# JonasGeiping/breaching

Measured on NVIDIA H100. Metric: reconstruction iters/sec (ResNet-18 224x224, invertinggradients), higher is better.
Workload: dtype tf32

## Files before the change

breaching_b200/csrc/igemm_tc.cu:

```cuda
#include <stdlib.h>
#include <string.h>

#include <array>
#include <map>
#include <mutex>
#include <type_traits>

#include <cuda.h>

#include "igemm.cuh"

namespace bre {

namespace {

constexpr int TC_BM = 128;
constexpr int TC_BK = 32;
constexpr int TC_STAGES = 4;
constexpr int TC_MAX_STAGES = 8;
constexpr int TC_THREADS = 128;
constexpr int TC_BLOCK = 2 * TC_THREADS;

struct TcDims {
  int M, Nc, K;
// ... 88 lines not shown
template <int N>
__device__ __forceinline__ void cp_async_wait() { asm volatile("cp.async.wait_group %0;" ::"n"(N) : "memory"); }
__device__ __forceinline__ void cp_async_arrive(uint64_t* bar) {
  asm volatile("cp.async.mbarrier.arrive.noinc.shared::cta.b64 [%0];" ::"r"(smem_u32(bar)) : "memory");
}
__device__ __forceinline__ void consumer_sync() { asm volatile("bar.sync 1, %0;" ::"n"(TC_THREADS) : "memory"); }
__device__ __forceinline__ void cluster_sync_all() {
  asm volatile("barrier.cluster.arrive.release.aligned;" ::: "memory");
  asm volatile("barrier.cluster.wait.acquire.aligned;" ::: "memory");
}
__device__ __forceinline__ float4 ld_dsmem4(uint32_t saddr, uint32_t rank) {
  uint32_t raddr;
  asm("mapa.shared::cluster.u32 %0, %1, %2;" : "=r"(raddr) : "r"(saddr), "r"(rank));
  float4 v;
  asm volatile("ld.shared::cluster.v4.f32 {%0, %1, %2, %3}, [%4];" : "=f"(v.x), "=f"(v.y), "=f"(v.z), "=f"(v.w) : "r"(raddr));
  return v;
}

struct TcMaps {
  CUtensorMap act[2];
  CUtensorMap wgt[2];
};

constexpr int TC_MAXCLS = 4;
struct ClsPlan {
  int ncls, stride;
  int tile0[TC_MAXCLS + 1];
  int Hc[TC_MAXCLS], Wc[TC_MAXCLS], y0[TC_MAXCLS], x0[TC_MAXCLS];
  int Ty[TC_MAXCLS], Tx[TC_MAXCLS], Ly[TC_MAXCLS], Lx[TC_MAXCLS], ey[TC_MAXCLS], ex[TC_MAXCLS];
};
struct TcMapsCls {
  CUtensorMap act[2 * TC_MAXCLS];
  CUtensorMap wgt[2];
};

__device__ __forceinline__ void mbar_expect_tx(uint64_t* bar, uint32_t bytes) {
  asm volatile("mbarrier.arrive.expect_tx.shared::cta.b64 _, [%0], %1;" ::"r"(smem_u32(bar)), "r"(bytes) : "memory");
}
__device__ __forceinline__ void tma_im2col(uint32_t dst, const CUtensorMap* tm, uint64_t* bar, int c, int w, int h, int n, int ow, int oh) {
  asm volatile(
      "cp.async.bulk.tensor.4d.shared::cluster.global.im2col.mbarrier::complete_tx::bytes [%0], [%1, {%3, %4, %5, %6}], [%2], {%7, %8};"
      ::"r"(dst), "l"(reinterpret_cast<uint64_t>(tm)), "r"(smem_u32(bar)), "r"(c), "r"(w), "r"(h), "r"(n), "h"((uint16_t)ow), "h"((uint16_t)oh)
      : "memory");
}
__device__ __forceinline__ void tma_tile2d(uint32_t dst, const CUtensorMap* tm, uint64_t* bar, int c0, int c1) {
  asm volatile("cp.async.bulk.tensor.2d.shared::cluster.global.tile.mbarrier::complete_tx::bytes [%0], [%1, {%3, %4}], [%2];"
               ::"r"(dst), "l"(reinterpret_cast<uint64_t>(tm)), "r"(smem_u32(bar)), "r"(c0), "r"(c1) : "memory");
}
__device__ __forceinline__ void tma_tile3d(uint32_t dst, const CUtensorMap* tm, uint64_t* bar, int c0, int c1, int c2) {
  asm volatile("cp.async.bulk.tensor.3d.shared::cluster.global.tile.mbarrier::complete_tx::bytes [%0], [%1, {%3, %4, %5}], [%2];"
               ::"r"(dst), "l"(reinterpret_cast<uint64_t>(tm)), "r"(smem_u32(bar)), "r"(c0), "r"(c1), "r"(c2) : "memory");
}

template <int NV>
__device__ __forceinline__ void fused_bnact(const GemmEpilogue& e, long long row, int n, float (&v)[NV]) {
  const long long o = row + n;
#pragma unroll
  for (int j = 0; j < NV; ++j) {
    float u = v[j];
    if (e.kind == 1) {
      if (e.has_bn) u = fmaf(u, __ldg(e.scale + n + j), __ldg(e.shift + n + j));
      if (e.res != nullptr) u += e.res[o + j];
      u = e.relu ? fmaxf(u, 0.f) : u;
      v[j] = e.round_out ? tf32_rna(u) : u;
    } else {
      if (e.has_bn) {
        const float xhat = fmaf(e.pre[o + j], __ldg(e.inv + n + j), __ldg(e.nrm + n + j));
        u = fmaf(__ldg(e.scale + n + j), u, fmaf(__ldg(e.v_gamma + n + j), xhat, __ldg(e.v_beta + n + j)));
      }
      if (e.res != nullptr) u += e.res[o + j];
      if (e.relu && !(e.post[o + j] > 0.f)) u = 0.f;
      v[j] = e.round_out ? tf32_rna(u) : u;
    }
  }
}

#ifdef BRE_TC_TRACE
__device__ long long g_tc_trace[16];
#define TC_MARK(i, cond) do { if ((cond) && blockIdx.x == 0 && blockIdx.y == 0 && blockIdx.z == 0) g_tc_trace[i] = clock64(); } while (0)
#else
#define TC_MARK(i, cond) do { } while (0)
#endif

template <int MODE, int BN, bool TMA, bool CLS = false>
__global__ void __launch_bounds__(TC_BLOCK) igemm_tc_kernel(GemmArgs a, TcDims d, int proxy_fence,
                                                            const __grid_constant__ std::conditional_t<CLS, TcMapsCls, TcMaps> maps, ClsPlan plan) {
  static_assert(!CLS || (MODE == GEMM_DGRAD && TMA), "per-class gathers: strided dgrad with the TMA producer only");
  constexpr uint32_t A_BYTES = TC_BM * TC_BK * 4, B_BYTES = BN * TC_BK * 4;
  extern __shared__ __align__(1024) uint8_t smem[];
  uint8_t* sA = smem;
  const int nst = 1 << d.stage_shift, stage_mask = nst - 1;
  uint8_t* sB = smem + nst * A_BYTES;
  __shared__ __align__(8) uint64_t bar_full[TC_MAX_STAGES];
  __shared__ __align__(8) uint64_t bar_empty[TC_MAX_STAGES];

  TC_MARK(0, threadIdx.x == 0);
  pdl_launch_dependents();
  const ConvGeom g = a.g;
  const int tid = threadIdx.x, warp = tid >> 5, lane = tid & 31;
  const int ptid = tid & (TC_THREADS - 1);
  const bool consumer = warp < TC_THREADS / 32;
  const int n0 = blockIdx.y * BN, z = blockIdx.z;
  int m0 = blockIdx.x * TC_BM;
  int kb_begin = z * d.kblocks_per_split;
  int kb_end = min(d.total_kblocks, kb_begin + d.kblocks_per_split);
  const int HoWo = g.Ho * g.Wo, HW = g.H * g.W;
  int cls = 0, cHc = 0, cWc = 0, cTy = 0, cTx = 0, cls_kps = 0, Mrows = d.M;
  if (CLS) {
#pragma unroll
    for (int c = 1; c < TC_MAXCLS; ++c)
      if (c < plan.ncls && (int)blockIdx.x >= plan.tile0[c]) cls = c;
    m0 = ((int)blockIdx.x - plan.tile0[cls]) * TC_BM;
    cHc = plan.Hc[cls]; cWc = plan.Wc[cls]; cTy = plan.Ty[cls]; cTx = plan.Tx[cls];
    Mrows = g.N * cHc * cWc;
    cls_kps = cTy * cTx * (g.Co / TC_BK);
    const int total = cls_kps * a.nsrc, per = (total + (int)gridDim.z - 1) / (int)gridDim.z;
    kb_begin = z * per;
    kb_end = min(total, kb_begin + per);
  }

  if (tid == 0) {
#pragma unroll
    for (int s = 0; s < TC_MAX_STAGES; ++s) { mbar_init(&bar_full[s], TMA ? 1 : TC_THREADS); mbar_init(&bar_empty[s], TC_THREADS / 32); }
    fence_barrier_init();
  }
  __syncthreads();
  TC_MARK(1, threadIdx.x == 0);

  constexpr bool a_mn = MODE == GEMM_WGRAD;
  constexpr bool b_mn = MODE != GEMM_FPROP;

  constexpr int A_VEC = TC_BM * TC_BK / 4 / TC_THREADS;
  constexpr int B_VEC = BN * TC_BK / 4 / TC_THREADS;
  const int gcol = ptid & 7, grow = (ptid >> 3) & 15;
  int a_off[A_VEC];
  unsigned long long a_taps[A_VEC];
  int a_yx[A_VEC];
  if (!TMA && !consumer && (MODE == GEMM_FPROP || MODE == GEMM_DGRAD)) {
#pragma unroll
    for (int j = 0; j < A_VEC; ++j) {
      const int m = m0 + grow + 16 * j;
      a_off[j] = 0; a_taps[j] = 0ull; a_yx[j] = 0;
      if (m < d.M) {
        if (MODE == GEMM_FPROP) {
          const int img = m / HoWo, rem = m - img * HoWo;
          const int p = rem / g.Wo, q = rem - p * g.Wo;
          const int y0 = p * g.stride - g.pad, x0 = q * g.stride - g.pad;
          a_off[j] = (int)(img * a.x_sN) + (y0 * g.W + x0) * a.x_sP + gcol * 4;
          for (int r = 0; r < g.R; ++r)
            for (int s2 = 0; s2 < g.S; ++s2)
              if (y0 + r >= 0 && y0 + r < g.H && x0 + s2 >= 0 && x0 + s2 < g.W) a_taps[j] |= 1ull << (r * g.S + s2);
        } else {
          const int img = m / HW, rem = m - img * HW;
          const int y = rem / g.W, x = rem - y * g.W;
          const int yb = y + g.pad, xb = x + g.pad;
          const int py = yb / g.stride, qx = xb / g.stride;
          const int ey = yb - py * g.stride, ex = xb - qx * g.stride;
          a_off[j] = ((img * g.Ho + py) * g.Wo + qx) * g.Co + gcol * 4;
          a_yx[j] = (ey << 16) | ex;
          for (int r = ey, pp = py; r < g.R; r += g.stride, --pp)
            for (int s2 = ex, qq = qx; s2 < g.S; s2 += g.stride, --qq)
              if (pp >= 0 && pp < g.Ho && qq >= 0 && qq < g.Wo) a_taps[j] |= 1ull << (r * g.S + s2);
        }
      }
    }
  }
  int it_src, it_rs, it_c0;
  {
    const int kch = (MODE == GEMM_DGRAD) ? g.Co : g.Ci;
    it_src = kb_begin / d.kblocks_per_src;
    const int kbase = (kb_begin - it_src * d.kblocks_per_src) * TC_BK;
    it_rs = (MODE == GEMM_WGRAD) ? 0 : kbase / kch;
    it_c0 = (MODE == GEMM_WGRAD) ? kbase : kbase - it_rs * kch;
  }

  const int nkb = kb_end > kb_begin ? kb_end - kb_begin : 0;
  int base_n = 0, base_h = 0, base_w = 0;
  if (CLS) {
    const int per = cHc * cWc;
    base_n = m0 / per;
    const int rem = m0 - base_n * per;
    const int iy0 = rem / cWc, ix0 = rem - iy0 * cWc;
    base_h = iy0 + plan.Ly[cls]; base_w = ix0 + plan.Lx[cls];
  } else if (TMA && MODE != GEMM_WGRAD) {
    const int per = (MODE == GEMM_FPROP) ? HoWo : HW, wid = (MODE == GEMM_FPROP) ? g.Wo : g.W;
    base_n = m0 / per;
// ... 129 lines not shown
    const uint32_t pa = smem_u32(sA + stage * A_BYTES), pb = smem_u32(sB + stage * B_BYTES);
    if (MODE == GEMM_FPROP) {
      const int r = it_rs / g.S, s = it_rs - r * g.S;
      const int tapoff = (r * g.W + s) * a.x_sP + it_c0;
#pragma unroll
      for (int j = 0; j < A_VEC; ++j) {
        const bool ok = (a_taps[j] >> it_rs) & 1ull;
        cp_async16(pa + off_k128(grow + 16 * j, gcol), ok ? act + (a_off[j] + tapoff) : act, ok ? 16u : 0u);
      }
      const float* q = wgt + (long long)(n0 + grow) * d.K + kbase + gcol * 4;
#pragma unroll
      for (int j = 0; j < B_VEC; ++j) cp_async16(pb + off_k128(grow + 16 * j, gcol), q + (long long)(16 * j) * d.K, 16u);
    } else if (MODE == GEMM_DGRAD) {
      const int rs = it_rs, k0 = it_c0;
      const int r = rs / g.S, s = rs - r * g.S;
      if (g.stride == 1) {
        const int tapoff = k0 - (r * g.Wo + s) * g.Co;
#pragma unroll
        for (int j = 0; j < A_VEC; ++j) {
          const bool ok = (a_taps[j] >> rs) & 1ull;
          cp_async16(pa + off_k128(grow + 16 * j, gcol), ok ? act + (a_off[j] + tapoff) : act, ok ? 16u : 0u);
        }
      } else {
        const bool st2 = g.stride == 2;
#pragma unroll
        for (int j = 0; j < A_VEC; ++j) {
          const bool ok = (a_taps[j] >> rs) & 1ull;
          const int dr = r - (a_yx[j] >> 16), ds = s - (a_yx[j] & 0xffff);
          const int tr = st2 ? dr >> 1 : dr / g.stride, ts = st2 ? ds >> 1 : ds / g.stride;
          cp_async16(pa + off_k128(grow + 16 * j, gcol), ok ? act + (a_off[j] + k0 - (tr * g.Wo + ts) * g.Co) : act, ok ? 16u : 0u);
        }
      }
      const int n4 = ptid & 15, kk = ptid >> 4;
#pragma unroll
      for (int j = 0; j < B_VEC; ++j) {
        const int k = kk + 8 * j;
        const float* gb = wgt + ((long long)(k0 + k) * (g.R * g.S) + rs) * g.Ci + n0 + n4 * 4;
        cp_async16(pb + off_mn128(4 * n4, k), gb, 16u);
      }
    } else {
      {
        const int m4 = ptid & 31, kk = ptid >> 5;
#pragma unroll
        for (int j = 0; j < A_VEC; ++j) {
          const int k = kk + 4 * j;
          const int pix = kbase + k;
          const bool kok = pix < d.K;
          const bool mok = kok && (m0 + m4 * 4 < d.M);
          const float* ga = mok ? wgt + (long long)pix * g.Co + m0 + m4 * 4 : wgt;
          cp_async16(pa + off_mn128(4 * m4, k), ga, mok ? 16u : 0u);
        }
      }
      {
        const int n4 = ptid & 15, kk = ptid >> 4;
        const int n = n0 + n4 * 4;
        const int rs = n / g.Ci, c = n - rs * g.Ci;
        const int r = rs / g.S, s = rs - r * g.S;
#pragma unroll
        for (int j = 0; j < B_VEC; ++j) {
          const int k = kk + 8 * j;
          const int pix = kbase + k;
          bool ok = pix < d.K;
          const float* gb = act;
          if (ok) {
            const int img = pix / HoWo, rem = pix - img * HoWo;
            const int p = rem / g.Wo, q = rem - p * g.Wo;
            const int h = p * g.stride - g.pad + r, w = q * g.stride - g.pad + s;
            ok = h >= 0 && h < g.H && w >= 0 && w < g.W;
            if (ok) gb = act + img * a.x_sN + (long long)(h * g.W + w) * a.x_sP + c;
          }
          cp_async16(pb + off_mn128(4 * n4, k), gb, ok ? 16u : 0u);
        }
      }
    }
    it_c0 += TC_BK;
    if (MODE == GEMM_WGRAD) {
      if (it_c0 >= d.kblocks_per_src * TC_BK) { it_c0 = 0; ++it_src; }
    } else if (it_c0 >= kch) {
      it_c0 = 0;
      if (++it_rs == g.R * g.S) { it_rs = 0; ++it_src; }
    }
  };

  float acc[2][BN / 2];
#pragma unroll
  for (int h = 0; h < 2; ++h)
#pragma unroll
    for (int i = 0; i < BN / 2; ++i) acc[h][i] = 0.f;
  const int gq = lane >> 2, tq = lane & 3;
  if (consumer) {
    for (int i = 0; i < nkb; ++i) {
      const int stage = i & stage_mask;
      mbar_wait(&bar_full[stage], (uint32_t)((i >> d.stage_shift) & 1));
      TC_MARK(4, i == 0 && tid == 0);
      if constexpr (MODE == GEMM_FPROP) {
        if (!TMA || (proxy_fence & 1)) fence_proxy_async();
        const uint32_t sa = smem_u32(sA) + stage * A_BYTES, sb = smem_u32(sB) + stage * B_BYTES;
        wgmma_fence();
#pragma unroll
        for (int j = 0; j < TC_BK / 8; ++j) {
          const uint64_t db = wgmma_desc_k128(sb + 32 * j);
          wgmma_tf32<BN>(acc[0], wgmma_desc_k128(sa + 32 * j), db);
          wgmma_tf32<BN>(acc[1], wgmma_desc_k128(sa + 64 * 128 + 32 * j), db);
        }
        wgmma_commit();
        wgmma_wait<1>();
        fence_regs(acc[0]);
        fence_regs(acc[1]);
        __syncwarp();
        if (i > 0 && lane == 0) mbar_arrive(&bar_empty[(i - 1) & stage_mask]);
      } else {
        const uint8_t* pa = sA + stage * A_BYTES;
        const uint8_t* pb = sB + stage * B_BYTES;
#pragma unroll
        for (int j = 0; j < TC_BK / 8; ++j) {
          const int k0 = 8 * j + tq;
          uint32_t af[2][4];
#pragma unroll
          for (int h = 0; h < 2; ++h) {
            const int r = 64 * h + 16 * warp + gq;
            af[h][0] = ld_op<a_mn>(pa, r, k0);
            af[h][1] = ld_op<a_mn>(pa, r + 8, k0);
            af[h][2] = ld_op<a_mn>(pa, r, k0 + 4);
            af[h][3] = ld_op<a_mn>(pa, r + 8, k0 + 4);
          }
#pragma unroll
          for (int jn = 0; jn < BN / 8; ++jn) {
            const uint32_t b0 = ld_op<b_mn>(pb, 8 * jn + gq, k0), b1 = ld_op<b_mn>(pb, 8 * jn + gq, k0 + 4);
            mma_tf32(&acc[0][4 * jn], af[0], b0, b1);
            mma_tf32(&acc[1][4 * jn], af[1], b0, b1);
          }
        }
        __syncwarp();
        if (lane == 0) mbar_arrive(&bar_empty[stage]);
      }
    }
    if constexpr (MODE == GEMM_FPROP) {
      wgmma_wait<0>();
      fence_regs(acc[0]);
      fence_regs(acc[1]);
    }
    TC_MARK(5, tid == 0);
  } else {
    if (TMA) {
      if (producer) {
        KbState st = pst;
        for (int i = pw; i < nkb; i += nprod) {
          const int stage = i & stage_mask;
          if (i >= nst) mbar_wait(&bar_empty[stage], (uint32_t)(((i >> d.stage_shift) - 1) & 1));
          if (i >= nst || !((pre_wgt >> i) & 1u)) {
            mbar_expect_tx(&bar_full[stage], A_BYTES + B_BYTES);
            issue_wgt_tma(stage, st);
          }
          issue_act_tma(stage, st);
          TC_MARK(3, i == (nkb < nst ? nkb : nst) - 1);
          for (int u = 0; u < nprod; ++u) kb_advance(st);
        }
      }
      __syncwarp();
    } else {
      for (int i = 0; i < nkb; ++i) {
        const int stage = i & stage_mask;
        if (i >= nst) mbar_wait(&bar_empty[stage], (uint32_t)(((i >> d.stage_shift) - 1) & 1));
        issue_block(stage);
        cp_async_arrive(&bar_full[stage]);
      }
      cp_async_wait<0>();
    }
  }

  const int splits = gridDim.z;
  auto out_row = [&](int mm, long long& row, int& cs) {
    if (CLS) {
      const int per = cHc * cWc;
      const int img = mm / per, rem = mm - img * per;
      const int iy = rem / cWc, ix = rem - iy * cWc;
      row = img * a.x_sN + (long long)((plan.y0[cls] + plan.stride * iy) * g.W + plan.x0[cls] + plan.stride * ix) * a.x_sP;
      cs = a.x_sC;
    } else if (MODE == GEMM_DGRAD) {
      const int img = mm / HW;
      row = img * a.x_sN + (long long)(mm - img * HW) * a.x_sP;
      cs = a.x_sC;
    } else {
      row = (long long)mm * d.Nc;
      cs = 1;
    }
  };
  if (consumer && splits == 1) {
#pragma unroll
    for (int h = 0; h < 2; ++h) {
#pragma unroll
      for (int hr = 0; hr < 2; ++hr) {
        const int mm = m0 + 64 * h + 16 * warp + gq + 8 * hr;
        if (mm >= Mrows) continue;
        long long row;
        int cs;
        out_row(mm, row, cs);
#pragma unroll
        for (int jn = 0; jn < BN / 8; ++jn) {
          const int n = n0 + 8 * jn + 2 * tq;
          float v[2] = {acc[h][4 * jn + 2 * hr], acc[h][4 * jn + 2 * hr + 1]};
          if (MODE == GEMM_FPROP && a.bias != nullptr) {
            v[0] += __ldg(a.bias + n);
            v[1] += __ldg(a.bias + n + 1);
          }
          float* op = a.out + row + (long long)n * cs;
          if (MODE == GEMM_FPROP && a.epi.kind != 0) {
            if (a.out != nullptr) *reinterpret_cast<float2*>(op) = make_float2(v[0], v[1]);
            fused_bnact<2>(a.epi, row, n, v);
            *reinterpret_cast<float2*>(a.epi.out2 + row + n) = make_float2(v[0], v[1]);
          } else if (cs == 1) {
            float2 t2 = make_float2(v[0], v[1]);
            if (a.accumulate) {
              const float2 o = *reinterpret_cast<const float2*>(op);
              t2.x += o.x; t2.y += o.y;
            }
            *reinterpret_cast<float2*>(op) = t2;
          } else {
#pragma unroll
            for (int j = 0; j < 2; ++j) {
              float* q = op + (long long)j * cs;
              *q = a.accumulate ? *q + v[j] : v[j];
            }
          }
        }
      }
    }
  } else if (consumer) {
    consumer_sync();
    float* part = reinterpret_cast<float*>(sA);
#pragma unroll
    for (int h = 0; h < 2; ++h) {
#pragma unroll
      for (int hr = 0; hr < 2; ++hr) {
        const int r = 64 * h + 16 * warp + gq + 8 * hr;
#pragma unroll
        for (int jn = 0; jn < BN / 8; ++jn) {
          const int c = 8 * jn + 2 * tq;
          const int chunk = (c >> 2) ^ (r & (BN / 4 - 1) & 15);
          *reinterpret_cast<float2*>(part + r * BN + chunk * 4 + (c & 3)) = make_float2(acc[h][4 * jn + 2 * hr], acc[h][4 * jn + 2 * hr + 1]);
        }
      }
    }
  }
  if (splits > 1) {
    TC_MARK(7, tid == 0);
    cluster_sync_all();
    TC_MARK(8, tid == 0);
    if (consumer) {
      auto reduce_rows = [&](auto s_tag) {
        constexpr int S = decltype(s_tag)::value;
        constexpr int C4 = BN / 4, SLOTS = (TC_BM / S) * C4 / TC_THREADS > 0 ? (TC_BM / S) * C4 / TC_THREADS : 1;
        const uint32_t part_s = smem_u32(sA);
        float4 t[SLOTS][S];
        int rr[SLOTS], cc[SLOTS];
#pragma unroll
        for (int sl = 0; sl < SLOTS; ++sl) {
          const int slot = tid + sl * TC_THREADS;
          rr[sl] = z * (TC_BM / S) + slot / C4;
          cc[sl] = slot % C4;
          const uint32_t local = part_s + (uint32_t)(rr[sl] * BN + ((cc[sl] ^ (rr[sl] & (BN / 4 - 1) & 15)) << 2)) * 4u;
#pragma unroll
          for (int q = 0; q < S; ++q) t[sl][q] = ld_dsmem4(local, (uint32_t)q);
        }
#pragma unroll
        for (int sl = 0; sl < SLOTS; ++sl) {
          const int r = rr[sl], c4 = cc[sl];
          if (m0 + r >= Mrows) continue;
          float4 acc4 = t[sl][0];
#pragma unroll
          for (int q = 1; q < S; ++q) { acc4.x += t[sl][q].x; acc4.y += t[sl][q].y; acc4.z += t[sl][q].z; acc4.w += t[sl][q].w; }
          const int n = n0 + c4 * 4;
          if (MODE == GEMM_FPROP && a.bias != nullptr) {
            acc4.x += __ldg(a.bias + n); acc4.y += __ldg(a.bias + n + 1); acc4.z += __ldg(a.bias + n + 2); acc4.w += __ldg(a.bias + n + 3);
          }
          long long row;
          int cs;
          out_row(m0 + r, row, cs);
          float* op = a.out + row + (long long)n * cs;
          if (MODE == GEMM_FPROP && a.epi.kind != 0) {
            if (a.out != nullptr) *reinterpret_cast<float4*>(op) = acc4;
            float vv[4] = {acc4.x, acc4.y, acc4.z, acc4.w};
            fused_bnact<4>(a.epi, row, n, vv);
            *reinterpret_cast<float4*>(a.epi.out2 + row + n) = make_float4(vv[0], vv[1], vv[2], vv[3]);
          } else if (cs == 1) {
            if (a.accumulate) {
              const float4 o = *reinterpret_cast<const float4*>(op);
              acc4.x += o.x; acc4.y += o.y; acc4.z += o.z; acc4.w += o.w;
            }
            *reinterpret_cast<float4*>(op) = acc4;
          } else {
            const float vv[4] = {acc4.x, acc4.y, acc4.z, acc4.w};
#pragma unroll
            for (int j = 0; j < 4; ++j) {
              float* qq = op + (long long)j * cs;
              *qq = a.accumulate ? *qq + vv[j] : vv[j];
            }
          }
        }
      };
      switch (splits) {
        case 2: reduce_rows(std::integral_constant<int, 2>{}); break;
        case 4: reduce_rows(std::integral_constant<int, 4>{}); break;
        default: reduce_rows(std::integral_constant<int, 8>{}); break;
      }
    }
    TC_MARK(9, tid == 0);
    cluster_sync_all();
  }
  TC_MARK(10, tid == 0);
}

inline bool aligned16(const void* p) { return (reinterpret_cast<uintptr_t>(p) & 15) == 0; }

typedef CUresult (*EncodeIm2colFn)(CUtensorMap*, CUtensorMapDataType, cuuint32_t, void*, const cuuint64_t*, const cuuint64_t*, const int*,
                                   const int*, cuuint32_t, cuuint32_t, const cuuint32_t*, CUtensorMapInterleave, CUtensorMapSwizzle,
                                   CUtensorMapL2promotion, CUtensorMapFloatOOBfill);
typedef CUresult (*EncodeTiledFn)(CUtensorMap*, CUtensorMapDataType, cuuint32_t, void*, const cuuint64_t*, const cuuint64_t*,
                                  const cuuint32_t*, const cuuint32_t*, CUtensorMapInterleave, CUtensorMapSwizzle,
                                  CUtensorMapL2promotion, CUtensorMapFloatOOBfill);

struct TmaApi {
  EncodeIm2colFn im2col = nullptr;
  EncodeTiledFn tiled = nullptr;
  int driver = 0;
  bool ok = false;
};
const TmaApi& tma_api() {
  static const TmaApi api = [] {
    TmaApi t;
    cudaDriverEntryPointQueryResult q;
    void* f = nullptr;
    if (cudaGetDriverEntryPoint("cuTensorMapEncodeIm2col", &f, cudaEnableDefault, &q) == cudaSuccess && q == cudaDriverEntryPointSuccess)
      t.im2col = reinterpret_cast<EncodeIm2colFn>(f);
    f = nullptr;
    if (cudaGetDriverEntryPoint("cuTensorMapEncodeTiled", &f, cudaEnableDefault, &q) == cudaSuccess && q == cudaDriverEntryPointSuccess)
      t.tiled = reinterpret_cast<EncodeTiledFn>(f);
    cudaDriverGetVersion(&t.driver);
    t.ok = t.im2col != nullptr && t.tiled != nullptr;
    return t;
  }();
  return api;
}

using MapKey = std::array<long long, 16>;
std::mutex g_map_mutex;
std::map<MapKey, CUtensorMap> g_map_cache;

bool im2col_map(CUtensorMap* out, const float* base, int N, int H, int W, int C, long long sN, int sP, int lower_w, int lower_h,
                int upper_w, int upper_h, int stride, int chans, int pixels, CUtensorMapSwizzle swz) {
  const MapKey key = {0, (long long)reinterpret_cast<uintptr_t>(base), N, H, W, C, sN, sP, lower_w, lower_h, upper_w, upper_h, stride, chans,
                      pixels, (long long)swz};
  std::lock_guard<std::mutex> lock(g_map_mutex);
  auto it = g_map_cache.find(key);
  if (it != g_map_cache.end()) { *out = it->second; return true; }
  const TmaApi& api = tma_api();
  if (!api.ok) return false;
  const cuuint64_t dims[4] = {(cuuint64_t)C, (cuuint64_t)W, (cuuint64_t)H, (cuuint64_t)N};
  const cuuint64_t strides[3] = {(cuuint64_t)sP * 4, (cuuint64_t)W * sP * 4, (cuuint64_t)sN * 4};
  const int lower[2] = {lower_w, lower_h}, upper[2] = {upper_w, upper_h};
  const cuuint32_t estr[4] = {1, (cuuint32_t)stride, (cuuint32_t)stride, 1};
  CUtensorMap tm;
  const CUresult res = api.im2col(&tm, CU_TENSOR_MAP_DATA_TYPE_FLOAT32, 4, const_cast<float*>(base), dims, strides, lower, upper,
                                  (cuuint32_t)chans, (cuuint32_t)pixels, estr, CU_TENSOR_MAP_INTERLEAVE_NONE, swz,
                                  CU_TENSOR_MAP_L2_PROMOTION_L2_128B, CU_TENSOR_MAP_FLOAT_OOB_FILL_NONE);
  if (res != CUDA_SUCCESS) return false;
  g_map_cache.emplace(key, tm);
  *out = tm;
  return true;
}

bool tiled_map(CUtensorMap* out, const float* base, int rank, const long long* dims_ll, const long long* strides_elems, const int* box_i,
               CUtensorMapSwizzle swz) {
  MapKey key = {1, (long long)reinterpret_cast<uintptr_t>(base), rank, (long long)swz};
  for (int i = 0; i < rank; ++i) { key[4 + i] = dims_ll[i]; key[8 + i] = box_i[i]; if (i + 1 < rank) key[12 + i] = strides_elems[i]; }
  std::lock_guard<std::mutex> lock(g_map_mutex);
  auto it = g_map_cache.find(key);
  if (it != g_map_cache.end()) { *out = it->second; return true; }
  const TmaApi& api = tma_api();
  if (!api.ok) return false;
  cuuint64_t dims[3], strides[2];
  cuuint32_t box[3], estr[3] = {1, 1, 1};
  for (int i = 0; i < rank; ++i) { dims[i] = (cuuint64_t)dims_ll[i]; box[i] = (cuuint32_t)box_i[i]; }
  for (int i = 0; i + 1 < rank; ++i) strides[i] = (cuuint64_t)strides_elems[i] * 4;
  CUtensorMap tm;
  const CUresult res = api.tiled(&tm, CU_TENSOR_MAP_DATA_TYPE_FLOAT32, (cuuint32_t)rank, const_cast<float*>(base), dims, strides, box, estr,
                                 CU_TENSOR_MAP_INTERLEAVE_NONE, swz, CU_TENSOR_MAP_L2_PROMOTION_L2_128B, CU_TENSOR_MAP_FLOAT_OOB_FILL_NONE);
  if (res != CUDA_SUCCESS) return false;
  g_map_cache.emplace(key, tm);
  *out = tm;
  return true;
}

bool tma_eligible(const GemmArgs& a) {
  static const int tma_env = [] { const char* e = getenv("BRE_TC_TMA"); return e ? atoi(e) : 1; }();
  if (!tma_env || !tma_api().ok) return false;
  const ConvGeom& g = a.g;
  if (g.stride > 8 || g.pad > 127 || g.R - 1 - g.pad > 127 || g.S - 1 - g.pad > 127 || g.R > 128 || g.S > 128) return false;
  if (a.mode == GEMM_DGRAD) return g.stride == 1;
  if (a.mode == GEMM_WGRAD) return g.Ci % 32 == 0;
  return true;
}

bool build_maps(const GemmArgs& a, int BN, TcMaps* maps) {
  const ConvGeom& g = a.g;
  const CUtensorMapSwizzle K128 = CU_TENSOR_MAP_SWIZZLE_128B;
  for (int s = 0; s < a.nsrc; ++s) {
    if (a.mode == GEMM_FPROP) {
      if (!im2col_map(&maps->act[s], a.act[s], g.N, g.H, g.W, g.Ci, a.x_sN, a.x_sP, -g.pad, -g.pad, g.pad - (g.S - 1), g.pad - (g.R - 1),
                      g.stride, TC_BK, TC_BM, K128))
        return false;
      const long long K = (long long)g.R * g.S * g.Ci;
      const long long dims[2] = {K, g.Co}, strides[1] = {K};
      const int box[2] = {TC_BK, BN};
      if (!tiled_map(&maps->wgt[s], a.wgt[s], 2, dims, strides, box, K128)) return false;
    } else if (a.mode == GEMM_DGRAD) {
      const int lw = g.pad - (g.S - 1), lh = g.pad - (g.R - 1);
      if (!im2col_map(&maps->act[s], a.act[s], g.N, g.Ho, g.Wo, g.Co, (long long)g.Ho * g.Wo * g.Co, g.Co, lw, lh, lw + g.W - g.Wo,
                      lh + g.H - g.Ho, 1, TC_BK, TC_BM, K128))
        return false;
      const long long dims[3] = {g.Ci, (long long)g.R * g.S, g.Co}, strides[2] = {g.Ci, (long long)g.R * g.S * g.Ci};
      const int box[3] = {32, 1, TC_BK};
      if (!tiled_map(&maps->wgt[s], a.wgt[s], 3, dims, strides, box, K128)) return false;
    } else {
      const long long npix = (long long)g.N * g.Ho * g.Wo;
      const long long dims[2] = {g.Co, npix}, strides[1] = {g.Co};
      const int box[2] = {32, TC_BK};
      if (!tiled_map(&maps->wgt[s], a.wgt[s], 2, dims, strides, box, K128)) return false;
      if (!im2col_map(&maps->act[s], a.act[s], g.N, g.H, g.W, g.Ci, a.x_sN, a.x_sP, -g.pad, -g.pad, g.pad - (g.S - 1), g.pad - (g.R - 1),
                      g.stride, 32, TC_BK, K128))
        return false;
    }
  }
  return true;
}

struct AxisPlan { bool any; int y0, Hc, T, L, U; };
inline AxisPlan axis_plan(int H, int Ho, int R, int stride, int pad, int e) {
  AxisPlan p{false, 0, 0, 0, 0, 0};
  p.y0 = ((e - pad) % stride + stride) % stride;
  if (p.y0 >= H) return p;
  p.any = true;
  p.Hc = (H - p.y0 + stride - 1) / stride;
  if (e >= R) return p;
  p.T = (R - e + stride - 1) / stride;
  const int c = (p.y0 + pad - e) / stride;
  p.L = c - (p.T - 1);
  p.U = p.Hc - Ho + p.L;
  return p;
}

bool cls_eligible(const GemmArgs& a) {
  static const int env = [] { const char* e = getenv("BRE_TC_STRIDED_TMA"); return e ? atoi(e) : 1; }();
  const ConvGeom& g = a.g;
  if (!env || a.mode != GEMM_DGRAD || g.stride != 2 || !tma_api().ok) return false;
  static const int tma_env = [] { const char* e = getenv("BRE_TC_TMA"); return e ? atoi(e) : 1; }();
  if (!tma_env || g.R > 16 || g.S > 16) return false;
  for (int ey = 0; ey < 2; ++ey)
    for (int horiz = 0; horiz < 2; ++horiz) {
      const AxisPlan p = horiz ? axis_plan(g.W, g.Wo, g.S, 2, g.pad, ey) : axis_plan(g.H, g.Ho, g.R, 2, g.pad, ey);
      if (p.any && p.T > 0 && (p.L < -128 || p.L > 127 || p.U < -128 || p.U > 127)) return false;
    }
  return true;
}

bool build_cls(const GemmArgs& a, ClsPlan* plan, TcMapsCls* maps) {
  const ConvGeom& g = a.g;
  memset(plan, 0, sizeof(*plan));
  plan->stride = g.stride;
  int tiles = 0, n = 0;
  for (int ey = 0; ey < g.stride; ++ey) {
    const AxisPlan py = axis_plan(g.H, g.Ho, g.R, g.stride, g.pad, ey);
    if (!py.any) continue;
    for (int ex = 0; ex < g.stride; ++ex) {
      const AxisPlan px = axis_plan(g.W, g.Wo, g.S, g.stride, g.pad, ex);
      if (!px.any) continue;
      if (n >= TC_MAXCLS) return false;
      const bool taps = py.T > 0 && px.T > 0;
      plan->Hc[n] = py.Hc; plan->Wc[n] = px.Hc; plan->y0[n] = py.y0; plan->x0[n] = px.y0;
      plan->Ty[n] = taps ? py.T : 0; plan->Tx[n] = taps ? px.T : 0;
      plan->Ly[n] = py.L; plan->Lx[n] = px.L; plan->ey[n] = ey; plan->ex[n] = ex;
      plan->tile0[n] = tiles;
      tiles += ceil_div((long long)g.N * py.Hc * px.Hc, TC_BM);
      for (int s = 0; s < a.nsrc && taps; ++s)
        if (!im2col_map(&maps->act[2 * n + s], a.act[s], g.N, g.Ho, g.Wo, g.Co, (long long)g.Ho * g.Wo * g.Co, g.Co, px.L, py.L, px.U, py.U, 1,
                        TC_BK, TC_BM, CU_TENSOR_MAP_SWIZZLE_128B))
          return false;
      if (!taps)
        for (int s = 0; s < a.nsrc; ++s) maps->act[2 * n + s] = maps->act[s];
      ++n;
    }
  }
  plan->ncls = n;
  plan->tile0[n] = tiles;
  for (int s = 0; s < a.nsrc; ++s) {
    const long long dims[3] = {g.Ci, (long long)g.R * g.S, g.Co}, strides[2] = {g.Ci, (long long)g.R * g.S * g.Ci};
    const int box[3] = {32, 1, TC_BK};
    if (!tiled_map(&maps->wgt[s], a.wgt[s], 3, dims, strides, box, CU_TENSOR_MAP_SWIZZLE_128B)) return false;
  }
  return n > 0;
}

template <int MODE, int BN, bool TMA, bool CLS = false>
int launch_tc(const GemmArgs& a, const TcDims& d0, const std::conditional_t<CLS, TcMapsCls, TcMaps>& maps, cudaStream_t stream,
              const ClsPlan* plan_in = nullptr) {
  TcDims d = d0;
  ClsPlan plan;
  memset(&plan, 0, sizeof(plan));
  if (CLS) plan = *plan_in;
  const int tm = CLS ? plan.tile0[plan.ncls] : ceil_div(d.M, TC_BM), tn = d.Nc / BN;
  if (CLS) {
    int kmax = 0;
    for (int c = 0; c < plan.ncls; ++c) kmax = kmax > plan.Ty[c] * plan.Tx[c] ? kmax : plan.Ty[c] * plan.Tx[c];
    d.total_kblocks = kmax * (a.g.Co / TC_BK) * a.nsrc;
    if (d.total_kblocks < 1) d.total_kblocks = 1;
  }
  const long long tiles = (long long)tm * tn;
  static const int max_splits_env = [] { const char* e = getenv("BRE_TC_MAX_SPLITS"); return e ? atoi(e) : 0; }();
  static const int target_ctas_env = [] { const char* e = getenv("BRE_TC_TARGET_CTAS"); return e ? atoi(e) : 0; }();
  const int target = target_ctas_env > 0 ? target_ctas_env : kNumSMs;
  constexpr int kMaxCluster = 8;
  int splits = a.splits;
  if (splits <= 0) {
    splits = 1;
    while (splits < kMaxCluster && tiles * splits < target && d.total_kblocks / (splits * 2) >= 2) splits *= 2;
  }
  if (max_splits_env > 0 && splits > max_splits_env) splits = max_splits_env;
  int pow2 = 1;
  while (pow2 * 2 <= splits && pow2 < kMaxCluster) pow2 *= 2;
  splits = pow2;
  while (splits > 1 && splits > d.total_kblocks) splits /= 2;
  d.kblocks_per_split = ceil_div(d.total_kblocks, splits);
  if (tn > 65535) { set_error("igemm_tc: grid too large"); return -1; }
  static const int stages_env = [] { const char* e = getenv("BRE_TC_STAGES"); return e ? atoi(e) : 0; }();
  static const int shortk_env = [] { const char* e = getenv("BRE_TC_SHORTK_STAGES"); return e ? atoi(e) : 2; }();
  const bool shortk = shortk_env == 2 && d.kblocks_per_split <= 6 && tm == 1 && tiles * splits > 2LL * kNumSMs;
  const int stages = (stages_env == 8 || stages_env == 2) ? stages_env : (shortk ? 2 : TC_STAGES);
  d.stage_shift = stages == 8 ? 3 : (stages == 2 ? 1 : 2);
  const size_t smem = (size_t)stages * (TC_BM + BN) * TC_BK * 4;
  const size_t smem_max = (size_t)TC_MAX_STAGES * (TC_BM + BN) * TC_BK * 4;
  static bool attr_done = false;
  if (!attr_done) {
    BRE_CUDA_CHECK(cudaFuncSetAttribute(igemm_tc_kernel<MODE, BN, TMA, CLS>, cudaFuncAttributeMaxDynamicSharedMemorySize, (int)smem_max));
    attr_done = true;
  }
  static const int proxy_fence_env = [] {
    const char* e = getenv("BRE_TC_PROXY_FENCE");
    const char* pf = getenv("BRE_TC_PREFETCH");
    const char* np = getenv("BRE_TC_PRODUCERS");
    int nprod = np ? atoi(np) : 2;
    if (nprod < 1 || nprod > 4) nprod = 2;
    return (e && atoi(e) ? 1 : 0) | ((pf ? atoi(pf) : 1) ? 2 : 0) | (nprod << 2);
  }();
  {
    cudaError_t lerr = launch_kernel(igemm_tc_kernel<MODE, BN, TMA, CLS>, dim3(tm, tn, splits), dim3(TC_BLOCK), smem, stream, splits, a, d,
                                     proxy_fence_env, maps, plan);
    if (lerr != cudaSuccess) { set_error(std::string("igemm_tc launch failed: ") + cudaGetErrorString(lerr)); return -2; }
  }
  BRE_CHECK_LAUNCH();
  return 0;
}

}

static bool narrow_tiles_ok(const GemmArgs& a) {
  static const int env = [] { const char* e = getenv("BRE_TC_NARROW"); return e ? atoi(e) : 1; }();
  if (!env || !tma_eligible(a)) return false;
  if (a.mode == GEMM_DGRAD && a.g.stride != 1) return false;
  if (a.mode == GEMM_WGRAD && (a.g.Ci % 32 != 0)) return false;
  return true;
}

bool igemm_tc_supported(const GemmArgs& a) {
  const ConvGeom& g = a.g;
  int M, Nc, K;
  gemm_dims(a, M, Nc, K);
  for (int s = 0; s < a.nsrc; ++s)
    if (!aligned16(a.act[s]) || !aligned16(a.wgt[s])) return false;
  if (!aligned16(a.out) || (a.splits == 0 && a.ws == nullptr)) return false;
  const bool x_nhwc = a.x_sC == 1 && a.x_sP % 4 == 0 && a.x_sN % 4 == 0;
  if (Nc % 64 != 0 && !(Nc % 32 == 0 && narrow_tiles_ok(a))) return false;
  switch (a.mode) {
    case GEMM_FPROP: return x_nhwc && g.Ci % TC_BK == 0 && g.R * g.S <= 64;
    case GEMM_DGRAD: return x_nhwc && g.Co % TC_BK == 0 && g.R * g.S <= 64;
    case GEMM_WGRAD: return x_nhwc && g.Co % 4 == 0 && g.Ci % 4 == 0 && g.R * g.S <= 64;
    default: return false;
  }
}

int launch_igemm_tc(const GemmArgs& a, cudaStream_t stream) {
  if (!igemm_tc_supported(a)) { set_error("igemm_tc: unsupported shape"); return -4; }
  TcDims d;
  gemm_dims(a, d.M, d.Nc, d.K);
  d.kblocks_per_src = ceil_div(d.K, TC_BK);
  d.total_kblocks = d.kblocks_per_src * a.nsrc;
  d.kblocks_per_split = d.total_kblocks;
  TcMaps maps;
  memset(&maps, 0, sizeof(maps));
  if (cls_eligible(a)) {
    ClsPlan plan;
    TcMapsCls cmaps;
    memset(&cmaps, 0, sizeof(cmaps));
    if (build_cls(a, &plan, &cmaps)) return launch_tc<GEMM_DGRAD, 64, true, true>(a, d, cmaps, stream, &plan);
  }
  const long long wide_tiles = (long long)ceil_div(d.M, TC_BM) * (d.Nc / 64);
  const bool underfilled = a.mode != GEMM_FPROP && d.Nc % 64 == 0 && wide_tiles * 16 <= kNumSMs && d.total_kblocks >= 64 &&
                           narrow_tiles_ok(a);
  if (d.Nc % 64 != 0 || (underfilled && build_maps(a, 32, &maps))) {
    if (d.Nc % 64 != 0 && !build_maps(a, 32, &maps)) { set_error("igemm_tc: tensor-map encoding failed for a narrow-tile shape"); return -4; }
    if (a.mode == GEMM_FPROP) return launch_tc<GEMM_FPROP, 32, true>(a, d, maps, stream);
    if (a.mode == GEMM_DGRAD) return launch_tc<GEMM_DGRAD, 32, true>(a, d, maps, stream);
    return launch_tc<GEMM_WGRAD, 32, true>(a, d, maps, stream);
  }
  const bool tma = tma_eligible(a) && build_maps(a, 64, &maps);
  if (a.mode == GEMM_FPROP) return tma ? launch_tc<GEMM_FPROP, 64, true>(a, d, maps, stream) : launch_tc<GEMM_FPROP, 64, false>(a, d, maps, stream);
  if (a.mode == GEMM_DGRAD) return tma ? launch_tc<GEMM_DGRAD, 64, true>(a, d, maps, stream) : launch_tc<GEMM_DGRAD, 64, false>(a, d, maps, stream);
  return tma ? launch_tc<GEMM_WGRAD, 64, true>(a, d, maps, stream) : launch_tc<GEMM_WGRAD, 64, false>(a, d, maps, stream);
}

}

#ifdef BRE_TC_TRACE
extern "C" int bre_debug_tc_trace(long long* out16) {
  return cudaMemcpyFromSymbol(out16, bre::g_tc_trace, sizeof(long long) * 16) == cudaSuccess ? 0 : -1;
}
#endif
```

Baseline: 671.8.

## Add 64-row tile variant for small-M fprop/dgrad with deeper pipelining

Templates the implicit-GEMM tensor-core kernel on the M tile size and adds a 64-row variant used when M is at most 64 for fprop and stride-1 dgrad on the TMA path. Half of each 128-row tile was padding for these small-M layers, so the change cuts wasted tensor-core work and shared-memory traffic. When the grid underfills the SMs and K is long, it also uses 8 pipeline stages. Producer count is clamped to the stage count, and split-K reduction slots are guarded for the smaller tile. The risks are more template instantiations and different occupancy and shared-memory use.

Measured after the change: 716.8 (median of 6 runs). +6.7%, better.

```diff
diff --git a/breaching_b200/csrc/igemm_tc.cu b/breaching_b200/csrc/igemm_tc.cu
--- a/breaching_b200/csrc/igemm_tc.cu
+++ b/breaching_b200/csrc/igemm_tc.cu
@@ -194,11 +194,13 @@
 #define TC_MARK(i, cond) do { } while (0)
 #endif
 
-template <int MODE, int BN, bool TMA, bool CLS = false>
+template <int MODE, int BN, bool TMA, bool CLS = false, int BM = TC_BM>
 __global__ void __launch_bounds__(TC_BLOCK) igemm_tc_kernel(GemmArgs a, TcDims d, int proxy_fence,
                                                             const __grid_constant__ std::conditional_t<CLS, TcMapsCls, TcMaps> maps, ClsPlan plan) {
   static_assert(!CLS || (MODE == GEMM_DGRAD && TMA), "per-class gathers: strided dgrad with the TMA producer only");
-  constexpr uint32_t A_BYTES = TC_BM * TC_BK * 4, B_BYTES = BN * TC_BK * 4;
+  static_assert(BM == TC_BM || (BM == 64 && TMA && !CLS && MODE != GEMM_WGRAD), "64-row tiles: fprop / stride-1 dgrad on the TMA producer");
+  constexpr int MH = BM / 64;
+  constexpr uint32_t A_BYTES = BM * TC_BK * 4, B_BYTES = BN * TC_BK * 4;
   extern __shared__ __align__(1024) uint8_t smem[];
   uint8_t* sA = smem;
   const int nst = 1 << d.stage_shift, stage_mask = nst - 1;
@@ -213,7 +215,7 @@
   const int ptid = tid & (TC_THREADS - 1);
   const bool consumer = warp < TC_THREADS / 32;
   const int n0 = blockIdx.y * BN, z = blockIdx.z;
-  int m0 = blockIdx.x * TC_BM;
+  int m0 = blockIdx.x * BM;
   int kb_begin = z * d.kblocks_per_split;
   int kb_end = min(d.total_kblocks, kb_begin + d.kblocks_per_split);
   const int HoWo = g.Ho * g.Wo, HW = g.H * g.W;
@@ -509,9 +511,9 @@
     }
   };
 
-  float acc[2][BN / 2];
-#pragma unroll
-  for (int h = 0; h < 2; ++h)
+  float acc[MH][BN / 2];
+#pragma unroll
+  for (int h = 0; h < MH; ++h)
 #pragma unroll
     for (int i = 0; i < BN / 2; ++i) acc[h][i] = 0.f;
   const int gq = lane >> 2, tq = lane & 3;
@@ -527,13 +529,13 @@
 #pragma unroll
         for (int j = 0; j < TC_BK / 8; ++j) {
           const uint64_t db = wgmma_desc_k128(sb + 32 * j);
-          wgmma_tf32<BN>(acc[0], wgmma_desc_k128(sa + 32 * j), db);
-          wgmma_tf32<BN>(acc[1], wgmma_desc_k128(sa + 64 * 128 + 32 * j), db);
+#pragma unroll
+          for (int h = 0; h < MH; ++h) wgmma_tf32<BN>(acc[h], wgmma_desc_k128(sa + h * 64 * 128 + 32 * j), db);
         }
         wgmma_commit();
         wgmma_wait<1>();
-        fence_regs(acc[0]);
-        fence_regs(acc[1]);
+#pragma unroll
+        for (int h = 0; h < MH; ++h) fence_regs(acc[h]);
         __syncwarp();
         if (i > 0 && lane == 0) mbar_arrive(&bar_empty[(i - 1) & stage_mask]);
       } else {
@@ -542,9 +544,9 @@
 #pragma unroll
         for (int j = 0; j < TC_BK / 8; ++j) {
           const int k0 = 8 * j + tq;
-          uint32_t af[2][4];
-#pragma unroll
-          for (int h = 0; h < 2; ++h) {
+          uint32_t af[MH][4];
+#pragma unroll
+          for (int h = 0; h < MH; ++h) {
             const int r = 64 * h + 16 * warp + gq;
             af[h][0] = ld_op<a_mn>(pa, r, k0);
             af[h][1] = ld_op<a_mn>(pa, r + 8, k0);
@@ -554,8 +556,8 @@
 #pragma unroll
           for (int jn = 0; jn < BN / 8; ++jn) {
             const uint32_t b0 = ld_op<b_mn>(pb, 8 * jn + gq, k0), b1 = ld_op<b_mn>(pb, 8 * jn + gq, k0 + 4);
-            mma_tf32(&acc[0][4 * jn], af[0], b0, b1);
-            mma_tf32(&acc[1][4 * jn], af[1], b0, b1);
+#pragma unroll
+            for (int h = 0; h < MH; ++h) mma_tf32(&acc[h][4 * jn], af[h], b0, b1);
           }
         }
         __syncwarp();
@@ -564,8 +566,8 @@
     }
     if constexpr (MODE == GEMM_FPROP) {
       wgmma_wait<0>();
-      fence_regs(acc[0]);
-      fence_regs(acc[1]);
+#pragma unroll
+      for (int h = 0; h < MH; ++h) fence_regs(acc[h]);
     }
     TC_MARK(5, tid == 0);
   } else {
@@ -615,7 +617,7 @@
   };
   if (consumer && splits == 1) {
 #pragma unroll
-    for (int h = 0; h < 2; ++h) {
+    for (int h = 0; h < MH; ++h) {
 #pragma unroll
       for (int hr = 0; hr < 2; ++hr) {
         const int mm = m0 + 64 * h + 16 * warp + gq + 8 * hr;
@@ -657,7 +659,7 @@
     consumer_sync();
     float* part = reinterpret_cast<float*>(sA);
 #pragma unroll
-    for (int h = 0; h < 2; ++h) {
+    for (int h = 0; h < MH; ++h) {
 #pragma unroll
       for (int hr = 0; hr < 2; ++hr) {
         const int r = 64 * h + 16 * warp + gq + 8 * hr;
@@ -677,15 +679,16 @@
     if (consumer) {
       auto reduce_rows = [&](auto s_tag) {
         constexpr int S = decltype(s_tag)::value;
-        constexpr int C4 = BN / 4, SLOTS = (TC_BM / S) * C4 / TC_THREADS > 0 ? (TC_BM / S) * C4 / TC_THREADS : 1;
+        constexpr int C4 = BN / 4, NSLOT = (BM / S) * C4, SLOTS = NSLOT / TC_THREADS > 0 ? NSLOT / TC_THREADS : 1;
         const uint32_t part_s = smem_u32(sA);
         float4 t[SLOTS][S];
         int rr[SLOTS], cc[SLOTS];
 #pragma unroll
         for (int sl = 0; sl < SLOTS; ++sl) {
           const int slot = tid + sl * TC_THREADS;
-          rr[sl] = z * (TC_BM / S) + slot / C4;
+          rr[sl] = z * (BM / S) + slot / C4;
           cc[sl] = slot % C4;
+          if (NSLOT < TC_THREADS && slot >= NSLOT) continue;
           const uint32_t local = part_s + (uint32_t)(rr[sl] * BN + ((cc[sl] ^ (rr[sl] & (BN / 4 - 1) & 15)) << 2)) * 4u;
 #pragma unroll
           for (int q = 0; q < S; ++q) t[sl][q] = ld_dsmem4(local, (uint32_t)q);
@@ -693,7 +696,7 @@
 #pragma unroll
         for (int sl = 0; sl < SLOTS; ++sl) {
           const int r = rr[sl], c4 = cc[sl];
-          if (m0 + r >= Mrows) continue;
+          if ((NSLOT < TC_THREADS && tid + sl * TC_THREADS >= NSLOT) || m0 + r >= Mrows) continue;
           float4 acc4 = t[sl][0];
 #pragma unroll
           for (int q = 1; q < S; ++q) { acc4.x += t[sl][q].x; acc4.y += t[sl][q].y; acc4.z += t[sl][q].z; acc4.w += t[sl][q].w; }
@@ -829,13 +832,13 @@
   return true;
 }
 
-bool build_maps(const GemmArgs& a, int BN, TcMaps* maps) {
+bool build_maps(const GemmArgs& a, int BN, TcMaps* maps, int BM = TC_BM) {
   const ConvGeom& g = a.g;
   const CUtensorMapSwizzle K128 = CU_TENSOR_MAP_SWIZZLE_128B;
   for (int s = 0; s < a.nsrc; ++s) {
     if (a.mode == GEMM_FPROP) {
       if (!im2col_map(&maps->act[s], a.act[s], g.N, g.H, g.W, g.Ci, a.x_sN, a.x_sP, -g.pad, -g.pad, g.pad - (g.S - 1), g.pad - (g.R - 1),
-                      g.stride, TC_BK, TC_BM, K128))
+                      g.stride, TC_BK, BM, K128))
         return false;
       const long long K = (long long)g.R * g.S * g.Ci;
       const long long dims[2] = {K, g.Co}, strides[1] = {K};
@@ -844,7 +847,7 @@
     } else if (a.mode == GEMM_DGRAD) {
       const int lw = g.pad - (g.S - 1), lh = g.pad - (g.R - 1);
       if (!im2col_map(&maps->act[s], a.act[s], g.N, g.Ho, g.Wo, g.Co, (long long)g.Ho * g.Wo * g.Co, g.Co, lw, lh, lw + g.W - g.Wo,
-                      lh + g.H - g.Ho, 1, TC_BK, TC_BM, K128))
+                      lh + g.H - g.Ho, 1, TC_BK, BM, K128))
         return false;
       const long long dims[3] = {g.Ci, (long long)g.R * g.S, g.Co}, strides[2] = {g.Ci, (long long)g.R * g.S * g.Ci};
       const int box[3] = {32, 1, TC_BK};
@@ -928,14 +931,14 @@
   return n > 0;
 }
 
-template <int MODE, int BN, bool TMA, bool CLS = false>
+template <int MODE, int BN, bool TMA, bool CLS = false, int BM = TC_BM>
 int launch_tc(const GemmArgs& a, const TcDims& d0, const std::conditional_t<CLS, TcMapsCls, TcMaps>& maps, cudaStream_t stream,
               const ClsPlan* plan_in = nullptr) {
   TcDims d = d0;
   ClsPlan plan;
   memset(&plan, 0, sizeof(plan));
   if (CLS) plan = *plan_in;
-  const int tm = CLS ? plan.tile0[plan.ncls] : ceil_div(d.M, TC_BM), tn = d.Nc / BN;
+  const int tm = CLS ? plan.tile0[plan.ncls] : ceil_div(d.M, BM), tn = d.Nc / BN;
   if (CLS) {
     int kmax = 0;
     for (int c = 0; c < plan.ncls; ++c) kmax = kmax > plan.Ty[c] * plan.Tx[c] ? kmax : plan.Ty[c] * plan.Tx[c];
@@ -962,13 +965,14 @@
   static const int stages_env = [] { const char* e = getenv("BRE_TC_STAGES"); return e ? atoi(e) : 0; }();
   static const int shortk_env = [] { const char* e = getenv("BRE_TC_SHORTK_STAGES"); return e ? atoi(e) : 2; }();
   const bool shortk = shortk_env == 2 && d.kblocks_per_split <= 6 && tm == 1 && tiles * splits > 2LL * kNumSMs;
-  const int stages = (stages_env == 8 || stages_env == 2) ? stages_env : (shortk ? 2 : TC_STAGES);
+  const bool deep = BM == 64 && tiles * splits <= kNumSMs && d.kblocks_per_split >= 16;
+  const int stages = (stages_env == 8 || stages_env == 2 || stages_env == 4) ? stages_env : (shortk ? 2 : (deep ? 8 : TC_STAGES));
   d.stage_shift = stages == 8 ? 3 : (stages == 2 ? 1 : 2);
-  const size_t smem = (size_t)stages * (TC_BM + BN) * TC_BK * 4;
-  const size_t smem_max = (size_t)TC_MAX_STAGES * (TC_BM + BN) * TC_BK * 4;
+  const size_t smem = (size_t)stages * (BM + BN) * TC_BK * 4;
+  const size_t smem_max = (size_t)TC_MAX_STAGES * (BM + BN) * TC_BK * 4;
   static bool attr_done = false;
   if (!attr_done) {
-    BRE_CUDA_CHECK(cudaFuncSetAttribute(igemm_tc_kernel<MODE, BN, TMA, CLS>, cudaFuncAttributeMaxDynamicSharedMemorySize, (int)smem_max));
+    BRE_CUDA_CHECK(cudaFuncSetAttribute(igemm_tc_kernel<MODE, BN, TMA, CLS, BM>, cudaFuncAttributeMaxDynamicSharedMemorySize, (int)smem_max));
     attr_done = true;
   }
   static const int proxy_fence_env = [] {
@@ -979,9 +983,11 @@
     if (nprod < 1 || nprod > 4) nprod = 2;
     return (e && atoi(e) ? 1 : 0) | ((pf ? atoi(pf) : 1) ? 2 : 0) | (nprod << 2);
   }();
+  int proxy_fence = proxy_fence_env;
+  if (((proxy_fence >> 2) & 7) > stages) proxy_fence = (proxy_fence & 3) | (stages << 2);
   {
-    cudaError_t lerr = launch_kernel(igemm_tc_kernel<MODE, BN, TMA, CLS>, dim3(tm, tn, splits), dim3(TC_BLOCK), smem, stream, splits, a, d,
-                                     proxy_fence_env, maps, plan);
+    cudaError_t lerr = launch_kernel(igemm_tc_kernel<MODE, BN, TMA, CLS, BM>, dim3(tm, tn, splits), dim3(TC_BLOCK), smem, stream, splits, a, d,
+                                     proxy_fence, maps, plan);
     if (lerr != cudaSuccess) { set_error(std::string("igemm_tc launch failed: ") + cudaGetErrorString(lerr)); return -2; }
   }
   BRE_CHECK_LAUNCH();
@@ -1033,11 +1039,20 @@
   const long long wide_tiles = (long long)ceil_div(d.M, TC_BM) * (d.Nc / 64);
   const bool underfilled = a.mode != GEMM_FPROP && d.Nc % 64 == 0 && wide_tiles * 16 <= kNumSMs && d.total_kblocks >= 64 &&
                            narrow_tiles_ok(a);
-  if (d.Nc % 64 != 0 || (underfilled && build_maps(a, 32, &maps))) {
-    if (d.Nc % 64 != 0 && !build_maps(a, 32, &maps)) { set_error("igemm_tc: tensor-map encoding failed for a narrow-tile shape"); return -4; }
-    if (a.mode == GEMM_FPROP) return launch_tc<GEMM_FPROP, 32, true>(a, d, maps, stream);
-    if (a.mode == GEMM_DGRAD) return launch_tc<GEMM_DGRAD, 32, true>(a, d, maps, stream);
+  static const int stream_env = [] { const char* e = getenv("BRE_TC_STREAM"); return e ? atoi(e) : 1; }();
+  const bool rows64 = stream_env && d.M <= 64 && (a.mode == GEMM_FPROP || a.mode == GEMM_DGRAD) && tma_eligible(a);
+  if (d.Nc % 64 != 0 || (underfilled && build_maps(a, 32, &maps, rows64 ? 64 : TC_BM))) {
+    if (d.Nc % 64 != 0 && !build_maps(a, 32, &maps, rows64 ? 64 : TC_BM)) {
+      set_error("igemm_tc: tensor-map encoding failed for a narrow-tile shape");
+      return -4;
+    }
+    if (a.mode == GEMM_FPROP) return rows64 ? launch_tc<GEMM_FPROP, 32, true, false, 64>(a, d, maps, stream) : launch_tc<GEMM_FPROP, 32, true>(a, d, maps, stream);
+    if (a.mode == GEMM_DGRAD) return rows64 ? launch_tc<GEMM_DGRAD, 32, true, false, 64>(a, d, maps, stream) : launch_tc<GEMM_DGRAD, 32, true>(a, d, maps, stream);
     return launch_tc<GEMM_WGRAD, 32, true>(a, d, maps, stream);
+  }
+  if (rows64 && build_maps(a, 64, &maps, 64)) {
+    if (a.mode == GEMM_FPROP) return launch_tc<GEMM_FPROP, 64, true, false, 64>(a, d, maps, stream);
+    return launch_tc<GEMM_DGRAD, 64, true, false, 64>(a, d, maps, stream);
   }
   const bool tma = tma_eligible(a) && build_maps(a, 64, &maps);
   if (a.mode == GEMM_FPROP) return tma ? launch_tc<GEMM_FPROP, 64, true>(a, d, maps, stream) : launch_tc<GEMM_FPROP, 64, false>(a, d, maps, stream);
```
